# yglbgyx/DS-GAN

Hardware: AMD Instinct MI355X
Metric: 256×256 paired imgs/sec (G+D step) at 1/2/4/8 MI355X; MS-SSIM Δ vs ref (higher is better)
Workload: dtype bf16; 1 GPU; DS-GAN optimize_parameters, MixConvNeXtML G + PatchGAN D + VGG16 perceptual + SSIM/L1/TV; global_batch=16, per_gpu_batch=16, parallelism=dp1, hip_graphs=True

## Files before the change

### ds-gan_amd/csrc/pconv.hip

```cpp
#include "common.h"
#include "lds_pitch.h"
#include <type_traits>
#include <stdlib.h>

namespace dsg {

typedef f32x16_t cf32x16;
typedef __attribute__((ext_vector_type(4))) unsigned int cu32x4;

struct PcArgs {
  const float* X; long x_bs;
  const unsigned short* Wb;
  float* Y; long y_bs;
  const float* bias;
  const float* gpre; long gpre_bs;
  int nb, K, M, H, W, Ho, Wo, pad;
  int tiles_w, tiles_h;
  int act, gact; float slope;
  int accumulate;
  float* ws; int kchunk;
};

constexpr int PC_STR = 40;

template <typename T16, int BM, int TH, int TW, int S, int KH, int KW>
__global__ __launch_bounds__(256, 2) void pconv_kernel(PcArgs g) {
  typedef hx8<T16> cbf16x8;
  constexpr int BN = TH * TW;
  static_assert(BN == 128, "128 output pixels per tile");
  constexpr int WM = 2, WN = 2, TM = BM / WM / 32, TN = BN / WN / 32;
  constexpr int PH = (TH - 1) * S + KH, PW = (TW - 1) * S + KW, PPIX = PH * PW;
  constexpr int PWP = S == 1 ? 32 : PW;
  static_assert(PWP >= PW, "patch pitch");
  constexpr int TAPS = KH * KW;
  constexpr int A_SZ = BM * PC_STR, P_SZ = PH * PWP * PC_STR;
  constexpr int A_ITEMS = BM * 4 / 256;
  constexpr int P_ITEMS = (PPIX * 4 + 255) / 256;
  __shared__ __attribute__((aligned(16))) T16 smem[2 * A_SZ + P_SZ];
  T16* Ps = smem + 2 * A_SZ;

  const int tid = threadIdx.x, lane = tid & 63, wave = __builtin_amdgcn_readfirstlane(tid >> 6);
  const int wm = wave / WN, wn = wave % WN;
  const int lr = lane & 31, lh = lane >> 5;

  const int mt = (g.M + BM - 1) / BM;
  int tile;
  {
    const int nwg = gridDim.x, id = blockIdx.x;
    const int xcd = id & 7, q = nwg >> 3, r = nwg & 7;
    tile = (xcd < r ? xcd * (q + 1) : r * (q + 1) + (xcd - r) * q) + (id >> 3);
  }
  const int m_t = tile % mt, rest0 = tile / mt;
  const int tpi = g.tiles_w * g.tiles_h;
  const int split = rest0 / (g.nb * tpi), rest = rest0 - split * (g.nb * tpi);
  const int bimg = rest / tpi, t_i = rest - bimg * tpi;
  const int m0 = m_t * BM;
  const int oh0 = (t_i / g.tiles_w) * TH, ow0 = (t_i % g.tiles_w) * TW;
  const int ih0 = oh0 * S - g.pad, iw0 = ow0 * S - g.pad;
  const int HW = g.H * g.W;
  const float* xb = g.X + (long)bimg * g.x_bs;

  int pbase[TN];
#pragma unroll
  for (int j = 0; j < TN; ++j) {
    const int n = wn * (BN / WN) + j * 32 + lr;
    pbase[j] = ((n / TW) * S * PWP + (n % TW) * S) * PC_STR + lh * 8;
  }

  cu32x4 ra[A_ITEMS];
  auto aload = [&](int tap, int k0) {
#pragma unroll
    for (int i = 0; i < A_ITEMS; ++i) {
      const int it = tid + i * 256, row = p80_row16(it), c8 = p80_slot16(it);
      const int m = m0 + row;
      ra[i] = m < g.M ? *reinterpret_cast<const cu32x4*>(g.Wb + ((long)tap * g.M + m) * g.K + k0 + c8 * 8)
                      : cu32x4{0u, 0u, 0u, 0u};
    }
  };
  auto astore = [&](int buf) {
    T16* As = smem + buf * A_SZ;
#pragma unroll
    for (int i = 0; i < A_ITEMS; ++i) {
      const int it = tid + i * 256;
      *reinterpret_cast<cu32x4*>(As + p80_row16(it) * PC_STR + p80_slot16(it) * 8) = ra[i];
    }
  };
  float rp[P_ITEMS][8];
  auto pload = [&](int k0) {
#pragma unroll
    for (int i = 0; i < P_ITEMS; ++i) {
      const int it = tid + i * 256;
      const int cg = it / PPIX, pix = it - cg * PPIX;
      const int pr = pix / PW, pc = pix - pr * PW;
      const int ih = ih0 + pr, iw = iw0 + pc;
      const bool in = it < PPIX * 4 && (unsigned)ih < (unsigned)g.H && (unsigned)iw < (unsigned)g.W;
      const float* src = xb + (long)(k0 + (in ? cg : 0) * 8) * HW + (in ? ih * g.W + iw : 0);
#pragma unroll
      for (int e = 0; e < 8; ++e) rp[i][e] = in ? src[(long)e * HW] : 0.f;
    }
  };
  auto pwrite = [&]() {
#pragma unroll
    for (int i = 0; i < P_ITEMS; ++i) {
      const int it = tid + i * 256;
      if (it < PPIX * 4) {
        const int cg = it / PPIX, pix = it - cg * PPIX;
        const int pr = pix / PW, pc = pix - pr * PW;
        cbf16x8 v;
#pragma unroll
        for (int e = 0; e < 8; ++e) v[e] = (T16)rp[i][e];
        *reinterpret_cast<cbf16x8*>(Ps + (pr * PWP + pc) * PC_STR + cg * 8) = v;
      }
    }
  };

  cf32x16 acc[TM][TN];
#pragma unroll
  for (int i = 0; i < TM; ++i) {
    float bv[16];
#pragma unroll
    for (int r = 0; r < 16; ++r) {
      const int m = m0 + wm * TM * 32 + i * 32 + (r & 3) + 8 * (r >> 2) + 4 * lh;
      bv[r] = (g.bias && !g.ws && m < g.M) ? g.bias[m] : 0.f;
    }
#pragma unroll
    for (int j = 0; j < TN; ++j)
#pragma unroll
      for (int r = 0; r < 16; ++r) acc[i][j][r] = bv[r];
  }

  const int kb0 = g.ws ? split * g.kchunk : 0;
  const int nkb = g.ws ? min(g.K / 32, kb0 + g.kchunk) : g.K / 32;
  int buf = 0;
  aload(0, kb0 * 32);
  pload(kb0 * 32);
  for (int kb = kb0; kb < nkb; ++kb) {
    const int k0 = kb * 32;
    __syncthreads();
    pwrite();
    astore(buf);
    __syncthreads();
    if (kb + 1 < nkb) pload(k0 + 32);
#pragma unroll 1
    for (int tap = 0; tap < TAPS; ++tap) {
      if (tap + 1 < TAPS) aload(tap + 1, k0);
      else if (kb + 1 < nkb) aload(0, k0 + 32);
      const T16* As = smem + buf * A_SZ;
      const int kh = tap / KW, kw = tap - (tap / KW) * KW;
      const int toff = (kh * PWP + kw) * PC_STR;
#pragma unroll
      for (int ks = 0; ks < 2; ++ks) {
        cbf16x8 af[TM], bfr[TN];
#pragma unroll
        for (int i = 0; i < TM; ++i)
          af[i] = *reinterpret_cast<const cbf16x8*>(As + (wm * TM * 32 + i * 32 + lr) * PC_STR + ks * 16 + lh * 8);
#pragma unroll
        for (int j = 0; j < TN; ++j)
          bfr[j] = *reinterpret_cast<const cbf16x8*>(Ps + pbase[j] + toff + ks * 16);
#pragma unroll
        for (int i = 0; i < TM; ++i)
#pragma unroll
          for (int j = 0; j < TN; ++j)
            acc[i][j] = mfma16(af[i], bfr[j], acc[i][j]);
      }
      if (tap + 1 < TAPS) {
        astore(buf ^ 1);
        __syncthreads();
        buf ^= 1;
      }
    }
  }

  const int HWo = g.Ho * g.Wo;
  if (g.ws) {
    float* wp = g.ws + ((long)split * g.nb + bimg) * g.M * HWo;
#pragma unroll
    for (int j = 0; j < TN; ++j) {
      const int n = wn * (BN / WN) + j * 32 + lr;
      const int oh = oh0 + n / TW, ow = ow0 + n % TW;
      if (oh >= g.Ho || ow >= g.Wo) continue;
      const long pofs = (long)oh * g.Wo + ow;
#pragma unroll
      for (int i = 0; i < TM; ++i)
#pragma unroll
        for (int r = 0; r < 16; ++r) {
          const int m = m0 + wm * TM * 32 + i * 32 + (r & 3) + 8 * (r >> 2) + 4 * lh;
          if (m < g.M) wp[(long)m * HWo + pofs] = acc[i][j][r];
        }
    }
    return;
  }
// ... 90 lines not shown
    for (long e = blockIdx.x * 256L + threadIdx.x; e < en.total; e += stride) Wb[e] = (T16)W[e];
    return;
  }
  const int Co = en.Co, Ci = en.Ci, KH = en.KH, KW = en.KW, mode = en.mode;
  const int M = mode == 0 ? Co : Ci, K = mode == 0 ? Ci : Co, T = KH * KW;
  const long pairs = (long)M * K, plane = pairs;
  for (long e = blockIdx.x * 256L + threadIdx.x; e < pairs; e += stride) {
    const int k = (int)(e % K), m = (int)(e / K);
    const int co = mode == 0 ? m : k, ci = mode == 0 ? k : m;
    const float* src = W + ((long)co * Ci + ci) * T;
    for (int tap = 0; tap < T; ++tap) {
      int kh = tap / KW, kw = tap - (tap / KW) * KW;
      if (mode == 1) { kh = KH - 1 - kh; kw = KW - 1 - kw; }
      Wb[(long)tap * plane + e] = (T16)src[kh * KW + kw];
    }
  }
}

constexpr int PC_TH = 8, PC_TW = 16;
static long pc_tiles(int nb, int M, int Ho, int Wo, int BM) {
  return (long)nb * ((Wo + PC_TW - 1) / PC_TW) * ((Ho + PC_TH - 1) / PC_TH) * ((M + BM - 1) / BM);
}

template <typename T16, int BM, int TH, int TW, int S, int KH, int KW>
static void pc_launch(PcArgs& g, int splits, hipStream_t st) {
  static_assert(TH == PC_TH && TW == PC_TW, "pc_tiles");
  g.tiles_w = (g.Wo + TW - 1) / TW;
  g.tiles_h = (g.Ho + TH - 1) / TH;
  const long tiles = pc_tiles(g.nb, g.M, g.Ho, g.Wo, BM);
  hipLaunchKernelGGL((pconv_kernel<T16, BM, TH, TW, S, KH, KW>), dim3((unsigned)(tiles * splits)), dim3(256), 0, st, g);
  if (splits > 1) {
    const long per = (long)g.nb * g.M * g.Ho * g.Wo;
    long blocks = (per + 255) / 256;
    if (blocks > 8192) blocks = 8192;
    hipLaunchKernelGGL(pconv_reduce_kernel, dim3((unsigned)blocks), dim3(256), 0, st, g, splits);
  }
}

template <typename T16, int BM>
static int pc_dispatch(PcArgs& g, int KH, int S, int splits, hipStream_t st) {
  if constexpr (BM <= 128) {
    if (KH == 3 && S == 1) { pc_launch<T16, BM, PC_TH, PC_TW, 1, 3, 3>(g, splits, st); return 0; }
    if (KH == 4 && S == 1) { pc_launch<T16, BM, PC_TH, PC_TW, 1, 4, 4>(g, splits, st); return 0; }
  }
  if (KH == 4 && S == 2) { pc_launch<T16, BM, PC_TH, PC_TW, 2, 4, 4>(g, splits, st); return 0; }
  return -1;
}

}

using namespace dsg;

extern "C" {

int dsgan_pconv_supported(int K, int KH, int KW, int stride) {
  if (K % 32 != 0 || K <= 0 || KH != KW) return 0;
  return (KH == 3 && stride == 1) || (KH == 4 && (stride == 1 || stride == 2));
}

int dsgan_conv_wtrans_bf16(const float* W, void* Wb, int Co, int Ci, int KH, int KW, int mode, hipStream_t st) {
  DSG_REQUIRE(W && Wb && mode >= 0 && mode <= 2, "dsgan_conv_wtrans_bf16: bad args");
  const long total = (long)KH * KW * Co * Ci;
  long blocks = (total + 255) / 256;
  if (blocks > 8192) blocks = 8192;
  with_half([&](auto* t_) {
    using T16 = std::remove_pointer_t<decltype(t_)>;
    hipLaunchKernelGGL((wtrans_bf16_kernel<T16>), dim3((unsigned)blocks), dim3(256), 0, st, W, (T16*)Wb, Co, Ci, KH, KW,
                       mode);
  });
  DSG_CHECK_LAUNCH();
  return 0;
}

int dsgan_wtrans_multi(const void* const* W, void* const* Wb, const int* desc, int n, hipStream_t st) {
  DSG_REQUIRE(W && Wb && desc && n >= 0, "dsgan_wtrans_multi: bad args");
  for (int i0 = 0; i0 < n; i0 += WT_MAXE) {
    WtList L{};
    const int ne = n - i0 < WT_MAXE ? n - i0 : WT_MAXE;
    long most = 1;
    for (int i = 0; i < ne; ++i) {
// ... 24 lines not shown

long dsgan_pconv_workspace(int nb, int K, int M, int Ho, int Wo) {
  if (K % 32 != 0 || K <= 0) return 0;
  const int bm = pc_bm(nb, M, Ho, Wo);
  int kc;
  const int S = max(pc_splits(pc_tiles(nb, M, Ho, Wo, bm), K / 32, &kc),
                    pc_splits(pc_tiles(nb, M, Ho, Wo, bm == 256 ? 128 : bm), K / 32, &kc));
  return S > 1 ? (long)S * nb * M * Ho * Wo : 0;
}

int dsgan_pconv_ws(const float* X, long x_bs, const void* Wb, const float* bias, float* Y, long y_bs,
                   const float* gpre, long gpre_bs, int nb, int K, int M, int H, int W, int Ho, int Wo,
                   int KH, int KW, int stride, int pad, int act, int gact, float slope, int accumulate,
                   float* ws, long ws_elems, hipStream_t st);

int dsgan_pconv(const float* X, long x_bs, const void* Wb, const float* bias, float* Y, long y_bs,
                const float* gpre, long gpre_bs, int nb, int K, int M, int H, int W, int Ho, int Wo,
                int KH, int KW, int stride, int pad, int act, int gact, float slope, int accumulate,
                hipStream_t st) {
  return dsgan_pconv_ws(X, x_bs, Wb, bias, Y, y_bs, gpre, gpre_bs, nb, K, M, H, W, Ho, Wo, KH, KW, stride, pad, act,
                        gact, slope, accumulate, nullptr, 0, st);
}

int dsgan_pconv_ws(const float* X, long x_bs, const void* Wb, const float* bias, float* Y, long y_bs,
                   const float* gpre, long gpre_bs, int nb, int K, int M, int H, int W, int Ho, int Wo,
                   int KH, int KW, int stride, int pad, int act, int gact, float slope, int accumulate,
                   float* ws, long ws_elems, hipStream_t st) {
  DSG_REQUIRE(X && Wb && Y && nb > 0 && M > 0 && Ho > 0 && Wo > 0, "dsgan_pconv: bad args");
  DSG_REQUIRE(dsgan_pconv_supported(K, KH, KW, stride), "dsgan_pconv: unsupported K=%d KH=%d KW=%d stride=%d", K, KH, KW, stride);
  DSG_REQUIRE(((uintptr_t)Wb & 15) == 0, "dsgan_pconv: Wb must be 16-byte aligned");
  DSG_REQUIRE((Ho - 1) * stride - pad + KH <= H + pad && (Wo - 1) * stride - pad + KW <= W + pad,
              "dsgan_pconv: output size inconsistent with input/pad");
  PcArgs g{};
  g.X = X; g.x_bs = x_bs; g.Wb = (const unsigned short*)Wb; g.Y = Y; g.y_bs = y_bs; g.bias = bias;
  g.gpre = gpre; g.gpre_bs = gpre_bs; g.nb = nb; g.K = K; g.M = M; g.H = H; g.W = W; g.Ho = Ho;
  g.Wo = Wo; g.pad = pad; g.act = act; g.gact = gact; g.slope = slope; g.accumulate = accumulate;
  const int bm0 = pc_bm(nb, M, Ho, Wo);
  const int bm = bm0 == 256 ? (stride == 2 ? 256 : 128) : bm0;
  int kc = 0;
  const int splits = ws ? pc_splits(pc_tiles(nb, M, Ho, Wo, bm), K / 32, &kc) : 1;
  g.ws = splits > 1 ? ws : nullptr;
  g.kchunk = kc;
  DSG_WS(splits > 1 ? (long)splits * nb * M * Ho * Wo : 0, ws, ws_elems, "dsgan_pconv (dsgan_pconv_workspace)");
  const int rc = with_half([&](auto* t_) {
    using T16 = std::remove_pointer_t<decltype(t_)>;
    return bm == 256 ? pc_dispatch<T16, 256>(g, KH, stride, splits, st)
           : bm == 128 ? pc_dispatch<T16, 128>(g, KH, stride, splits, st)
                       : pc_dispatch<T16, 64>(g, KH, stride, splits, st);
  });
  DSG_REQUIRE(rc == 0, "dsgan_pconv: no kernel for KH=%d stride=%d", KH, stride);
  DSG_CHECK_LAUNCH();
  return 0;
}

}
```

### ds-gan_amd/dsgan_hip/_lib.py

```python
import ctypes
import os

import torch

_HERE = os.path.dirname(os.path.abspath(__file__))
LIB_PATH = os.environ.get("DSGAN_HIP_LIB", os.path.join(_HERE, "libdsgan_hip.so"))

P = ctypes.c_void_p
L = ctypes.c_long
I = ctypes.c_int
F = ctypes.c_float
D = ctypes.c_double
S = ctypes.c_void_p

SIGNATURES = {
    "dsgan_abi_version": [],
    "dsgan_set_half_type": [ctypes.c_int],
    "dsgan_amp_parts": [],
    "dsgan_amp_check": [P, L, P, P, F, F, I, S],
    "dsgan_adam_amp": [P, P, P, P, L, D, D, D, D, P, S],
    "dsgan_get_half_type": [],
    "dsgan_clear_launch_error": [],
    "dsgan_ktimer": [I],
    "dsgan_ktimer_read": [P, I],
# ... 14 lines not shown
    "dsgan_pw_dgrad_io_ws": [P, I, P, L, I, P, L, I, P, L, I, I, I, I, I, P, L, S],
    "dsgan_pw_fd_workspace": [I, I, I, I, I],
    "dsgan_wtrans_multi": [P, P, P, I, S],
    "dsgan_pw_tune": [I, I],
    "dsgan_pw_f32_supported": [I, I, I, I, L, L, P, P],
    "dsgan_pw_f32_wgrad_workspace": [I, I, I, I],
    "dsgan_pw_gemm_f32": [I, P, L, P, L, P, L, P, P, L, I, I, I, I, I, I, I, I, F, P, L, S],
    "dsgan_mlp_supported": [I, I, I],
    "dsgan_mlp_fwd": [P, L, I, P, P, P, P, P, L, I, I, I, I, I, S],
    "dsgan_mlp_bwd": [P, L, I, P, L, P, P, P, P, L, P, P, P, I, I, I, I, S],
    "dsgan_mlp_wgrad_workspace": [I, I, I, I],
    "dsgan_mlp_wgrad": [P, L, I, P, L, P, P, P, P, P, P, P, L, I, I, I, I, S],
    "dsgan_mlp_tune": [I, I],
    "dsgan_colsum": [P, I, I, P, S],
    "dsgan_split_defer": [I],
    "dsgan_split_pending": [],
    "dsgan_split_flush": [S],
    "dsgan_f32_to_bf16": [P, P, L, S],
    "dsgan_pconv_supported": [I, I, I, I],
    "dsgan_conv_wtrans_bf16": [P, P, I, I, I, I, I, S],
    "dsgan_pconv": [P, L, P, P, P, L, P, L] + [I] * 13 + [F, I, S],
    "dsgan_pconv_workspace": [I] * 5,
    "dsgan_pconv_ws": [P, L, P, P, P, L, P, L] + [I] * 13 + [F, I, P, L, S],
    "dsgan_pw_small_supported": [I, I, I, L, L],
    "dsgan_pw_small": [P, L, P, I, I, P, P, L, P, L] + [I] * 8 + [F, S],
    "dsgan_pw_small2": [P, L, P, I, I, P, L, P, I, P, P, L, P, L] + [I] * 8 + [F, S],
    "dsgan_pconvt_supported": [I, I, I, I],
    "dsgan_pconvt": [P, L, P, P, P, L, P, L] + [I] * 11 + [F, I, S],
    "dsgan_wconv_supported": [I, I, I, I],
    "dsgan_wconv_workspace": [I, I, I, I, I, I, I],
    "dsgan_wconv": [P, L, P, L, P, P, L] + [I] * 11 + [S],
    "dsgan_wconv_db": [P, L, P, L, P, P, P, L] + [I] * 11 + [S],
    "dsgan_wconv_xh": [P, L, P, L, P, P, L] + [I] * 11 + [S],
    "dsgan_conv_wtrans": [P, P, I, I, I, I, I, I, I, I, I, S],
    "dsgan_tconv": [P, L, P, P, P, L, P, L] + [I] * 9 + [P, P] + [I] * 7 + [F, S],
    "dsgan_tconv_workspace": [I] * 6,
    "dsgan_tconv_ws": [P, L, P, P, P, L, P, L] + [I] * 9 + [P, P] + [I] * 7 + [F, I, P, L, S],
    "dsgan_tconv_ws_xh": [P, L, P, P, P, L, P, L] + [I] * 9 + [P, P] + [I] * 7 + [F, P, L, S],
    "dsgan_conv_small_out": [P, L, P, L, L, L, L, P, P, L] + [I] * 13 + [S],
    "dsgan_conv_small_in": [P, L, P, L, L, L, L, P, P, L] + [I] * 13 + [F, I, S],
    "dsgan_conv_wgrad_small_workspace": [I] * 7,
    "dsgan_conv_wgrad_small": [P, L, P, L, P] + [I] * 11 + [P, L, S],
    "dsgan_thin3_supported": [I, I, I, L, L],
    "dsgan_pgstem_supported": [I] * 4,
    "dsgan_pgstem_fwd": [P, L, P, P, P, L] + [I] * 5 + [F, S],
    "dsgan_pgstem_wgrad_workspace": [I] * 5,
# ... 123 lines not shown
```

### ds-gan_amd/dsgan_hip/functional.py

```python
import contextlib
import os
import math

import ctypes

import torch

from . import _lib
from ._lib import call, ptr, stream


def wsa(t):
    if t is not None and _DEFER_KEEP[0] is not None:
        _DEFER_CAND.append(t)
    return (ptr(t), t.numel() if t is not None else 0)


DEFER_SPLITS = [os.environ.get("DSGAN_DEFER_SPLITS", "1") != "0"]
_DEFER_KEEP = [None]
_DEFER_CAND = []


def _defer_hook(queued):
    if queued and _DEFER_KEEP[0] is not None:
# ... 334 lines not shown
            and bool(_lib.load().dsgan_pw_small_supported(K, M, P, xbs, ybs)))


PGLAST = [True]


def _pglast_ok(Cout, Cin, KH, KW, stride, pad, H, W, w):
    return (PGLAST[0] and Cout == 1 and KH == 4 and KW == 4 and stride == 1 and pad == 1 and w.dim() == 4
            and w.is_contiguous() and bool(_lib.load().dsgan_pglast_supported(Cin, H, W)))


def _thin3_ok(M, H, W, bs_small, bs_big, t_small, t_big):
    return (t_small.data_ptr() % 16 == 0 and t_big.data_ptr() % 16 == 0
            and bool(_lib.load().dsgan_thin3_supported(M, H, W, bs_small, bs_big)))


def _pconv_ok(K, KH, KW, stride):
    return _is16() and bool(_lib.load().dsgan_pconv_supported(K, KH, KW, stride))


def _pconv(x, xbs, wb, b, y, ybs, N, K, M, H, W, Ho, Wo, KH, KW, stride, pad, act, gpre, gbs, gact, accumulate):
    nws = _lib.load().dsgan_pconv_workspace(N, K, M, Ho, Wo)
    ws = torch.empty(nws, device=x.device, dtype=torch.float32) if nws > 0 else None
    call("dsgan_pconv_ws", ptr(x), xbs, ptr(wb), ptr(b), ptr(y), ybs, ptr(gpre), gbs, N, K, M, H, W, Ho, Wo, KH, KW,
         stride, pad, ACT[act], ACT[gact], LRELU_SLOPE, int(accumulate), *wsa(ws), stream())


def conv_fwd_raw(x, w, b, stride, pad, act=None, out=None, pre=None, accumulate=False, xact=None):
    x, xbs = nchw(x)
    N, Cin, H, W = x.shape
    Cout, Cin_w, KH, KW = w.shape if w.dim() == 4 else (w.shape[0], w.shape[1], 1, 1)
    if Cin_w != Cin:
        raise ValueError("conv: input has %d channels, weight expects %d" % (Cin, Cin_w))
    Ho = (H + 2 * pad - KH) // stride + 1
    Wo = (W + 2 * pad - KW) // stride + 1
    y = out if out is not None else _empty(N, Cout, Ho, Wo, x)
    y, ybs = nchw(y)
    pbs = 0
    if pre is not None:
        pre, pbs = nchw(pre)
    e0 = IGEMM_TIMER.begin()
    fam = "igemm_kernel"
    if (KH == 3 and KW == 3 and stride == 1 and pad == 1 and act is None and pre is None and xact is None
            and w.is_contiguous() and _thin3_ok(Cout, H, W, ybs, xbs, y, x)):
        fam = "thin3_kernel"
        call("dsgan_thin3_fwd", ptr(x), xbs, ptr(w), ptr(b), ptr(y), ybs, N, Cin, Cout, H, W, int(accumulate),
             stream())
    elif KH == 1 and KW == 1 and stride == 1 and pad == 0 and pre is None and _pws_ok(Cin, Cout, H * W, xbs, ybs, x, y):
# ... 8 lines not shown
    elif Cout <= 8 and act is None and pre is None and xact is None:
        fam = "small_out_kernel"
        call("dsgan_conv_small_out", ptr(x), xbs, ptr(w), Cin * KH * KW, KH * KW, KW, 1, ptr(b), ptr(y), ybs,
             N, Cin, Cout, H, W, Ho, Wo, KH, KW, stride, pad, 0, int(accumulate), stream())
    elif Cin * KH * KW <= 36 and Cout >= 16 and pre is None and xact is None and act in (None, "relu", "lrelu"):
        fam = "small_in_kernel"
        call("dsgan_conv_small_in", ptr(x), xbs, ptr(w), Cin * KH * KW, KH * KW, KW, 1, ptr(b), ptr(y), ybs,
             N, Cin, Cout, H, W, Ho, Wo, KH, KW, stride, pad, 0, ACT[act], LRELU_SLOPE, int(accumulate), stream())
    elif KH == 1 and KW == 1 and stride == 1 and pad == 0 and _pw_ok(0, Cout, Cin, H * W, 0, xbs, w.data_ptr(), x.data_ptr()):
        fam = "pwgemm_kernel"
        if xact is None and _pw_io_ok(Cin, H * W, xbs, ybs, x, y, pre, pbs):
            call("dsgan_pw_fwd_io_ws", ptr(bf16_weight(w)), 1, ptr(x), xbs, 0, ptr(y), ybs, 0, ptr(pre), pbs, 0,
                 ptr(b), Cout, Cin, H * W, N, ACT[act], int(accumulate), LRELU_SLOPE,
                 *wsa(_pw_fd_ws(0, Cout, Cin, H * W, N, x)), stream())
        else:
            call("dsgan_pw_gemm", 0, ptr(w), 0, ptr(x), xbs, ptr(y), ybs, ptr(b), ptr(pre), pbs, None, 0,
                 Cout, N * H * W, Cin, H * W, N, ACT[act], 0, ACT[xact], int(accumulate), LRELU_SLOPE,
                 *wsa(_pw_fd_ws(0, Cout, Cin, H * W, N, x)), stream())
    elif (KH == 1 and KW == 1 and stride == 1 and pad == 0 and pre is None and xact is None
          and _pwf_ok(0, Cout, Cin, H * W, 0, xbs, w.data_ptr(), x.data_ptr())):
        fam = "pwf32_kernel"
        call("dsgan_pw_gemm_f32", 0, ptr(w), 0, ptr(x), xbs, ptr(y), ybs, ptr(b), None, 0, Cout, N * H * W, Cin,
             H * W, N, ACT[act], 0, int(accumulate), LRELU_SLOPE, None, 0, stream())
    elif w.dim() == 4 and pre is None and xact is None and _pconv_ok(Cin, KH, KW, stride):
        fam = "pconv_kernel"
        _pconv(x, xbs, _wtrans_bf16(w, 0), b, y, ybs, N, Cin, Cout, H, W, Ho, Wo, KH, KW, stride, pad, act,
               None, 0, None, accumulate)
    elif (_is16() and w.dim() == 4 and (KH > 1 or KW > 1) and Cin % 32 == 0
          and pre is None and not accumulate and xact is None and KH * KW <= 16):
        fam = "tconv_kernel"
        wt = _wtrans_bf16(w, 0) if Cin % 8 == 0 else _wtrans(w, 0)
        taps = [(kh - pad, kw - pad) for kh in range(KH) for kw in range(KW)]
        _tconv(x, xbs, wt, b, y, ybs, None, 0, N, Cin, Cout, H, W, Ho, Wo, stride, taps, Ho, Wo, 1, 0, 0,
               act, None)
    else:
        call("dsgan_conv_fwd", ptr(x), xbs, ptr(w), ptr(b), ptr(y), ybs, ptr(pre), pbs, N, Cin, H, W,
             Cout, KH, KW, stride, pad, Ho, Wo, ACT[act], LRELU_SLOPE, int(accumulate), ACT[xact], _prec(),
             stream())
    IGEMM_TIMER.end(e0, _conv_flops(N, Cin, Cout, KH, KW, Ho, Wo), ("fwd", N, Cin, H, W, Cout, KH, stride), fam,
                    _nb(x, w, b, y, pre) + (_nb(y) if accumulate else 0.0))
    return y


def conv_dgrad_raw(dy, w, x_shape, stride, pad, bias=None, act=None, gpre=None, gact=None,
                   out=None, accumulate=False):
    dy, dybs = nchw(dy)
    N, Cin, H, W = x_shape
# ... 981 lines not shown
            res = None
        else:
            x, w, t, mean, rstd, res = ctx.saved_tensors
        N, Ci, Hi, Wi = x.shape
        Co, H, W = t.shape[1], t.shape[2], t.shape[3]
        HW = H * W
        dyt, dybs = nchw(dy[:, :Co] if ctx.cat else dy)
        t4, tbs = nchw(t)
        rbs = 0
        if res is not None:
            res, rbs = nchw(res)
        want_dres = res is not None and ctx.needs_input_grad[3]
        dres = _empty(N, Co, H, W, t) if want_dres else None
        dth = torch.empty((N, Co, H, W), device=t.device, dtype=half_dtype())
        psum = torch.empty(N * Co, device=t.device, dtype=torch.float32)
        e0 = AUX_TIMER.begin()
        call("dsgan_instnorm_bwd_h", ptr(dyt), dybs, ptr(t4), tbs, ptr(res), rbs, ptr(mean), ptr(rstd), ptr(dth),
             Co * HW, ptr(psum), ptr(dres), Co * HW, N, Co, HW, _in_act(ctx.act), LRELU_SLOPE, IN_EPS, stream())
        AUX_TIMER.end(e0, 0.0, ("in_bwd_h", N, Co, H, W, ctx.act, res is not None), "instnorm",
                      _nb(dyt, t4, res, dres) + _nb(dth))
        dx = None
        if ctx.needs_input_grad[0]:
            dx = _empty(N, Ci, Hi, Wi, x)
            taps = [(kh - 1, kw - 1) for kh in range(3) for kw in range(3)]
            dh = (ctypes.c_int * 9)(*[q[0] for q in taps])
            dw = (ctypes.c_int * 9)(*[q[1] for q in taps])
            nws = _lib.load().dsgan_tconv_workspace(N, Co, Ci, Hi, Wi, 9)
            ws = torch.empty(nws, device=t.device, dtype=torch.float32) if nws > 0 else None
            e0 = IGEMM_TIMER.begin()
            call("dsgan_tconv_ws_xh", ptr(dth), Co * HW, ptr(_wtrans_bf16(w, 0)), None, ptr(dx), Ci * Hi * Wi, None,
                 0, N, Co, Ci, H, W, Hi, Wi, 2, 9, ctypes.cast(dh, ctypes.c_void_p), ctypes.cast(dw, ctypes.c_void_p),
                 Hi, Wi, 1, 0, 0, 0, 0, LRELU_SLOPE, *wsa(ws), stream())
            IGEMM_TIMER.end(e0, _conv_flops(N, Co, Ci, 3, 3, Hi, Wi), ("fwd", N, Co, H, W, Ci, 3, 2), "tconv_kernel",
                            _nb(dth, dx) + 2.0 * w.numel())
        gw = _grad_buf(ctx.w_ref) if ctx.needs_input_grad[1] else None
        if gw is not None:
            x4, xbs = nchw(x)
            ws = torch.empty(_lib.load().dsgan_wconv_workspace(N, Co, Ci, Hi, Wi, 3, 3), device=t.device,
                             dtype=torch.float32)
            e0 = IGEMM_TIMER.begin()
            call("dsgan_wconv_xh", ptr(x4), xbs, ptr(dth), Co * HW, ptr(gw), *wsa(ws), N, Co, Ci, H, W, Hi, Wi, 3, 3,
                 2, 1, stream())
            IGEMM_TIMER.end(e0, _conv_flops(N, Co, Ci, 3, 3, Hi, Wi), ("wgrad", N, Co, H, W, Ci, 3, 2), "wconv_kernel",
                            _nb(x4, dth, gw))
        gb = _grad_buf(ctx.b_ref) if (ctx.has_b and ctx.needs_input_grad[2]) else None
        if gb is not None:
# ... 674 lines not shown
```

### include/dsgan_hip.h

```cpp
#ifndef DSGAN_HIP_H
#define DSGAN_HIP_H

#include <hip/hip_runtime.h>

#ifdef __cplusplus
extern "C" {
#endif

int dsgan_abi_version(void);
const char* dsgan_last_error_string(void);
int dsgan_set_plan_only(int on);
long dsgan_last_ws_need(void);
int dsgan_set_half_type(int t);
int dsgan_get_half_type(void);
int dsgan_clear_launch_error(void);
int dsgan_ktimer(int on);
int dsgan_ktimer_read(float* ms, int max);

int dsgan_conv_fwd(const float* x, long x_bs, const float* w, const float* bias, float* y,
                   long y_bs, float* ypre, long ypre_bs, int N, int Cin, int H, int W, int Cout,
                   int KH, int KW, int stride, int pad, int Ho, int Wo, int act, float slope,
                   int accumulate, int xact, int prec, hipStream_t stream);
int dsgan_conv_dgrad(const float* dy, long dy_bs, const float* w, const float* bias, float* dx,
                     long dx_bs, float* ypre, long ypre_bs, const float* gpre, long gpre_bs,
// ... 109 lines not shown
                   const float* gpre, long gpre_bs, int nb, int K, int M, int Hin, int Win, int Hout,
                   int Wout, int stride, int ntaps, const int* dh, const int* dw, int Hdst, int Wdst,
                   int os, int ph, int pw, int act, int gact, float slope, int wt_bf16, float* ws,
                   long ws_elems, hipStream_t stream);
int dsgan_tconv_ws_xh(const void* Xh, long x_bs, const void* Wt, const float* bias, float* Y, long y_bs,
                      const float* gpre, long gpre_bs, int nb, int K, int M, int Hin, int Win, int Hout,
                      int Wout, int stride, int ntaps, const int* dh, const int* dw, int Hdst, int Wdst,
                      int os, int ph, int pw, int act, int gact, float slope, float* ws, long ws_elems,
                      hipStream_t stream);

int dsgan_pconv_supported(int K, int KH, int KW, int stride);
int dsgan_conv_wtrans_bf16(const float* W, void* Wb, int Co, int Ci, int KH, int KW, int mode,
                           hipStream_t stream);
int dsgan_wtrans_multi(const void* const* W, void* const* Wb, const int* desc, int n, hipStream_t stream);
int dsgan_pconv(const float* X, long x_bs, const void* Wb, const float* bias, float* Y, long y_bs,
                const float* gpre, long gpre_bs, int nb, int K, int M, int H, int W, int Ho, int Wo,
                int KH, int KW, int stride, int pad, int act, int gact, float slope, int accumulate,
                hipStream_t stream);
long dsgan_pconv_workspace(int nb, int K, int M, int Ho, int Wo);
int dsgan_pconv_ws(const float* X, long x_bs, const void* Wb, const float* bias, float* Y, long y_bs,
                   const float* gpre, long gpre_bs, int nb, int K, int M, int H, int W, int Ho, int Wo,
                   int KH, int KW, int stride, int pad, int act, int gact, float slope, int accumulate,
                   float* ws, long ws_elems, hipStream_t stream);

int dsgan_pw_small_supported(int K, int M, int P, long x_bs, long y_bs);
int dsgan_pw_small(const float* X, long x_bs, const float* W, int wm, int wk, const float* bias, float* Y,
                   long y_bs, const float* G, long g_bs, int nb, int K, int M, int P, int act, int xact,
                   int gact, int accumulate, float slope, hipStream_t stream);
int dsgan_pw_small2(const float* X, long x_bs, const float* W, int wm, int wk, const float* X2,
                    long x2_bs, const float* W2, int K2, const float* bias, float* Y, long y_bs,
                    const float* G, long g_bs, int nb, int K, int M, int P, int act, int xact, int gact,
                    int accumulate, float slope, hipStream_t stream);

int dsgan_pconvt_supported(int K, int KS, int stride, int pad);
int dsgan_pconvt(const float* X, long x_bs, const void* Wb, const float* bias, float* Y, long y_bs,
                 const float* gpre, long gpre_bs, int nb, int K, int M, int Hi, int Wi, int Ho, int Wo,
                 int KS, int stride, int pad, int gact, float slope, int accumulate, hipStream_t stream);

int dsgan_wconv_supported(int C, int KH, int KW, int stride);
long dsgan_wconv_workspace(int nb, int C, int M, int Ho, int Wo, int KH, int KW);
int dsgan_wconv(const float* D, long d_bs, const float* X, long x_bs, float* dw, float* ws, long ws_elems,
                int nb, int C, int M, int H, int W, int Ho, int Wo, int KH, int KW, int stride, int pad,
                hipStream_t stream);
int dsgan_wconv_db(const float* D, long d_bs, const float* X, long x_bs, float* dw, float* db, float* ws,
                   long ws_elems, int nb, int C, int M, int H, int W, int Ho, int Wo, int KH, int KW, int stride,
                   int pad, hipStream_t stream);
// ... 152 lines not shown
```

Before: 651.1 img/s.

## Add 3x3 stride-2 patch-conv path with 16-bit vectorized input staging

Extends the patch-tile implicit-GEMM conv kernel to 3x3 stride-2 convolutions, and routes the conv-transpose data-gradient and eligible forward 3x3/s2 convs through it. A new 16-bit input variant stages rows with 128-bit vector loads and register shuffles instead of per-element gathers. A three-deep register ring prefetches weight slices across taps, with the unrolled tap loop. The aim is to replace the slower generic tap-gather path and cut global load instruction count, at the cost of more registers and template instantiations.

```diff
diff --git a/ds-gan_amd/csrc/pconv.hip b/ds-gan_amd/csrc/pconv.hip
--- a/ds-gan_amd/csrc/pconv.hip
+++ b/ds-gan_amd/csrc/pconv.hip
@@ -9,7 +9,7 @@
 typedef __attribute__((ext_vector_type(4))) unsigned int cu32x4;
 
 struct PcArgs {
-  const float* X; long x_bs;
+  const void* X; long x_bs;
   const unsigned short* Wb;
   float* Y; long y_bs;
   const float* bias;
@@ -23,9 +23,11 @@
 
 constexpr int PC_STR = 40;
 
-template <typename T16, int BM, int TH, int TW, int S, int KH, int KW>
+template <typename T16, int BM, int TH, int TW, int S, int KH, int KW, bool XH = false, bool VEC = false>
 __global__ __launch_bounds__(256, 2) void pconv_kernel(PcArgs g) {
   typedef hx8<T16> cbf16x8;
+  typedef std::conditional_t<XH, unsigned short, float> XT;
+  static_assert(!VEC || (XH && S == 2 && KH == 3 && KW == 3 && TW == 16), "row staging: 16-bit 3x3 stride 2");
   constexpr int BN = TH * TW;
   static_assert(BN == 128, "128 output pixels per tile");
   constexpr int WM = 2, WN = 2, TM = BM / WM / 32, TN = BN / WN / 32;
@@ -36,6 +38,8 @@
   constexpr int A_SZ = BM * PC_STR, P_SZ = PH * PWP * PC_STR;
   constexpr int A_ITEMS = BM * 4 / 256;
   constexpr int P_ITEMS = (PPIX * 4 + 255) / 256;
+  constexpr int V_ITEMS = (PH * 32 + 255) / 256;
+  constexpr int GI = VEC ? 1 : P_ITEMS, VI = VEC ? V_ITEMS : 1;
   __shared__ __attribute__((aligned(16))) T16 smem[2 * A_SZ + P_SZ];
   T16* Ps = smem + 2 * A_SZ;
 
@@ -58,7 +62,7 @@
   const int oh0 = (t_i / g.tiles_w) * TH, ow0 = (t_i % g.tiles_w) * TW;
   const int ih0 = oh0 * S - g.pad, iw0 = ow0 * S - g.pad;
   const int HW = g.H * g.W;
-  const float* xb = g.X + (long)bimg * g.x_bs;
+  const XT* xb = (const XT*)g.X + (long)bimg * g.x_bs;
 
   int pbase[TN];
 #pragma unroll
@@ -67,51 +71,120 @@
     pbase[j] = ((n / TW) * S * PWP + (n % TW) * S) * PC_STR + lh * 8;
   }
 
-  cu32x4 ra[A_ITEMS];
-  auto aload = [&](int tap, int k0) {
+  constexpr int AD = VEC ? 3 : 1;
+  static_assert(TAPS % AD == 0 && TAPS > AD, "slice ring");
+  cu32x4 ra[AD][A_ITEMS];
+  auto aload_s = [&](int slot, int tap, int k0) {
 #pragma unroll
     for (int i = 0; i < A_ITEMS; ++i) {
       const int it = tid + i * 256, row = p80_row16(it), c8 = p80_slot16(it);
       const int m = m0 + row;
-      ra[i] = m < g.M ? *reinterpret_cast<const cu32x4*>(g.Wb + ((long)tap * g.M + m) * g.K + k0 + c8 * 8)
-                      : cu32x4{0u, 0u, 0u, 0u};
-    }
-  };
-  auto astore = [&](int buf) {
+      ra[slot][i] = m < g.M ? *reinterpret_cast<const cu32x4*>(g.Wb + ((long)tap * g.M + m) * g.K + k0 + c8 * 8)
+                            : cu32x4{0u, 0u, 0u, 0u};
+    }
+  };
+  auto astore_s = [&](int buf, int slot) {
     T16* As = smem + buf * A_SZ;
 #pragma unroll
     for (int i = 0; i < A_ITEMS; ++i) {
       const int it = tid + i * 256;
-      *reinterpret_cast<cu32x4*>(As + p80_row16(it) * PC_STR + p80_slot16(it) * 8) = ra[i];
-    }
-  };
-  float rp[P_ITEMS][8];
-  auto pload = [&](int k0) {
-#pragma unroll
-    for (int i = 0; i < P_ITEMS; ++i) {
+      *reinterpret_cast<cu32x4*>(As + p80_row16(it) * PC_STR + p80_slot16(it) * 8) = ra[slot][i];
+    }
+  };
+  auto aload = [&](int tap, int k0) { aload_s(0, tap, k0); };
+  auto astore = [&](int buf) { astore_s(buf, 0); };
+  XT rp[GI][8];
+  auto pload_g = [&](int k0) {
+#pragma unroll
+    for (int i = 0; i < GI; ++i) {
       const int it = tid + i * 256;
       const int cg = it / PPIX, pix = it - cg * PPIX;
       const int pr = pix / PW, pc = pix - pr * PW;
       const int ih = ih0 + pr, iw = iw0 + pc;
       const bool in = it < PPIX * 4 && (unsigned)ih < (unsigned)g.H && (unsigned)iw < (unsigned)g.W;
-      const float* src = xb + (long)(k0 + (in ? cg : 0) * 8) * HW + (in ? ih * g.W + iw : 0);
-#pragma unroll
-      for (int e = 0; e < 8; ++e) rp[i][e] = in ? src[(long)e * HW] : 0.f;
-    }
-  };
-  auto pwrite = [&]() {
-#pragma unroll
-    for (int i = 0; i < P_ITEMS; ++i) {
+      const XT* src = xb + (long)(k0 + (in ? cg : 0) * 8) * HW + (in ? ih * g.W + iw : 0);
+#pragma unroll
+      for (int e = 0; e < 8; ++e) rp[i][e] = in ? src[(long)e * HW] : (XT)0;
+    }
+  };
+  auto pwrite_g = [&]() {
+#pragma unroll
+    for (int i = 0; i < GI; ++i) {
       const int it = tid + i * 256;
       if (it < PPIX * 4) {
         const int cg = it / PPIX, pix = it - cg * PPIX;
         const int pr = pix / PW, pc = pix - pr * PW;
         cbf16x8 v;
 #pragma unroll
-        for (int e = 0; e < 8; ++e) v[e] = (T16)rp[i][e];
+        for (int e = 0; e < 8; ++e) {
+          if constexpr (XH) v[e] = __builtin_bit_cast(T16, rp[i][e]);
+          else v[e] = (T16)rp[i][e];
+        }
         *reinterpret_cast<cbf16x8*>(Ps + (pr * PWP + pc) * PC_STR + cg * 8) = v;
       }
     }
+  };
+  cu32x4 rv[VI][4];
+  unsigned short rl[4];
+  auto pload_v = [&](int k0) {
+#pragma unroll
+    for (int i = 0; i < VI; ++i) {
+      const int it = tid + i * 256;
+      const int c = it & 3, cg = (it >> 2) & 7, pr = it >> 5;
+      const int ih = ih0 + pr, iw = iw0 + 1 + 8 * c;
+      const bool in = pr < PH && (unsigned)ih < (unsigned)g.H && iw < g.W;
+      const XT* src = xb + (long)(k0 + cg * 4) * HW + (in ? ih * g.W + iw : 0);
+#pragma unroll
+      for (int e = 0; e < 4; ++e)
+        rv[i][e] = in ? *reinterpret_cast<const cu32x4*>(src + (long)e * HW) : cu32x4{0u, 0u, 0u, 0u};
+    }
+    {
+      const int cg = tid & 7, pr = tid >> 3;
+      const int ih = ih0 + pr;
+      const bool in = pr < PH && (unsigned)ih < (unsigned)g.H && iw0 >= 0;
+      const XT* src = xb + (long)(k0 + cg * 4) * HW + (in ? ih * g.W + iw0 : 0);
+#pragma unroll
+      for (int e = 0; e < 4; ++e) rl[e] = in ? src[(long)e * HW] : (XT)0;
+    }
+  };
+  auto pwrite_v = [&]() {
+    typedef __attribute__((ext_vector_type(2))) unsigned int cu32x2;
+#pragma unroll
+    for (int i = 0; i < VI; ++i) {
+      const int it = tid + i * 256;
+      const int c = it & 3, cg = (it >> 2) & 7, pr = it >> 5;
+      if (pr < PH) {
+        cu32x4 r[4];
+#pragma unroll
+        for (int e = 0; e < 4; ++e) {
+          const cu32x4 u = rv[i][e];
+          const cu32x4 t = (c & 1) ? cu32x4{u[1], u[2], u[3], u[0]} : u;
+          r[e] = (c & 2) ? cu32x4{t[2], t[3], t[0], t[1]} : t;
+        }
+        T16* row = Ps + (pr * PWP + 1 + 8 * c) * PC_STR + cg * 4;
+#pragma unroll
+        for (int d = 0; d < 4; ++d) {
+          T16* dst = row + 2 * ((d + c) & 3) * PC_STR;
+          *reinterpret_cast<cu32x2*>(dst) =
+              cu32x2{(r[0][d] & 0xffffu) | (r[1][d] << 16), (r[2][d] & 0xffffu) | (r[3][d] << 16)};
+          *reinterpret_cast<cu32x2*>(dst + PC_STR) =
+              cu32x2{(r[0][d] >> 16) | (r[1][d] & 0xffff0000u), (r[2][d] >> 16) | (r[3][d] & 0xffff0000u)};
+        }
+      }
+    }
+    if (tid < PH * 8) {
+      const int cg = tid & 7, pr = tid >> 3;
+      *reinterpret_cast<cu32x2*>(Ps + pr * PWP * PC_STR + cg * 4) =
+          cu32x2{(unsigned)rl[0] | ((unsigned)rl[1] << 16), (unsigned)rl[2] | ((unsigned)rl[3] << 16)};
+    }
+  };
+  auto pload = [&](int k0) {
+    if constexpr (VEC) pload_v(k0);
+    else pload_g(k0);
+  };
+  auto pwrite = [&]() {
+    if constexpr (VEC) pwrite_v();
+    else pwrite_g();
   };
 
   cf32x16 acc[TM][TN];
@@ -132,41 +205,72 @@
   const int kb0 = g.ws ? split * g.kchunk : 0;
   const int nkb = g.ws ? min(g.K / 32, kb0 + g.kchunk) : g.K / 32;
   int buf = 0;
-  aload(0, kb0 * 32);
-  pload(kb0 * 32);
-  for (int kb = kb0; kb < nkb; ++kb) {
-    const int k0 = kb * 32;
-    __syncthreads();
-    pwrite();
-    astore(buf);
-    __syncthreads();
-    if (kb + 1 < nkb) pload(k0 + 32);
+  auto tap_mma = [&](int tap) {
+    const T16* As = smem + buf * A_SZ;
+    const int kh = tap / KW, kw = tap - (tap / KW) * KW;
+    const int toff = (kh * PWP + kw) * PC_STR;
+#pragma unroll
+    for (int ks = 0; ks < 2; ++ks) {
+      cbf16x8 af[TM], bfr[TN];
+#pragma unroll
+      for (int i = 0; i < TM; ++i)
+        af[i] = *reinterpret_cast<const cbf16x8*>(As + (wm * TM * 32 + i * 32 + lr) * PC_STR + ks * 16 + lh * 8);
+#pragma unroll
+      for (int j = 0; j < TN; ++j)
+        bfr[j] = *reinterpret_cast<const cbf16x8*>(Ps + pbase[j] + toff + ks * 16);
+#pragma unroll
+      for (int i = 0; i < TM; ++i)
+#pragma unroll
+        for (int j = 0; j < TN; ++j)
+          acc[i][j] = mfma16(af[i], bfr[j], acc[i][j]);
+    }
+  };
+  if constexpr (AD > 1) {
+    constexpr int PT = TAPS - 1 - AD - 1;
+#pragma unroll
+    for (int s = 0; s < AD; ++s) aload_s(s, s, kb0 * 32);
+    pload(kb0 * 32);
+    for (int kb = kb0; kb < nkb; ++kb) {
+      const int k0 = kb * 32;
+      __syncthreads();
+      pwrite();
+      astore_s(buf, 0);
+      __syncthreads();
+      aload_s(0, AD, k0);
+#pragma unroll
+      for (int tap = 0; tap < TAPS; ++tap) {
+        tap_mma(tap);
+        if (tap + 1 < TAPS) {
+          const int slot = (tap + 1) % AD, nt = tap + 1 + AD;
+          astore_s(buf ^ 1, slot);
+          if (nt < TAPS) aload_s(slot, nt, k0);
+          if (tap == PT && kb + 1 < nkb) pload(k0 + 32);
+          if (nt >= TAPS && kb + 1 < nkb) aload_s(slot, nt - TAPS, k0 + 32);
+          __syncthreads();
+          buf ^= 1;
+        }
+      }
+    }
+  } else {
+    aload(0, kb0 * 32);
+    pload(kb0 * 32);
+    for (int kb = kb0; kb < nkb; ++kb) {
+      const int k0 = kb * 32;
+      __syncthreads();
+      pwrite();
+      astore(buf);
+      __syncthreads();
+      if (kb + 1 < nkb) pload(k0 + 32);
 #pragma unroll 1
-    for (int tap = 0; tap < TAPS; ++tap) {
-      if (tap + 1 < TAPS) aload(tap + 1, k0);
-      else if (kb + 1 < nkb) aload(0, k0 + 32);
-      const T16* As = smem + buf * A_SZ;
-      const int kh = tap / KW, kw = tap - (tap / KW) * KW;
-      const int toff = (kh * PWP + kw) * PC_STR;
-#pragma unroll
-      for (int ks = 0; ks < 2; ++ks) {
-        cbf16x8 af[TM], bfr[TN];
-#pragma unroll
-        for (int i = 0; i < TM; ++i)
-          af[i] = *reinterpret_cast<const cbf16x8*>(As + (wm * TM * 32 + i * 32 + lr) * PC_STR + ks * 16 + lh * 8);
-#pragma unroll
-        for (int j = 0; j < TN; ++j)
-          bfr[j] = *reinterpret_cast<const cbf16x8*>(Ps + pbase[j] + toff + ks * 16);
-#pragma unroll
-        for (int i = 0; i < TM; ++i)
-#pragma unroll
-          for (int j = 0; j < TN; ++j)
-            acc[i][j] = mfma16(af[i], bfr[j], acc[i][j]);
-      }
-      if (tap + 1 < TAPS) {
-        astore(buf ^ 1);
-        __syncthreads();
-        buf ^= 1;
+      for (int tap = 0; tap < TAPS; ++tap) {
+        if (tap + 1 < TAPS) aload(tap + 1, k0);
+        else if (kb + 1 < nkb) aload(0, k0 + 32);
+        tap_mma(tap);
+        if (tap + 1 < TAPS) {
+          astore(buf ^ 1);
+          __syncthreads();
+          buf ^= 1;
+        }
       }
     }
   }
@@ -303,13 +407,14 @@
   return (long)nb * ((Wo + PC_TW - 1) / PC_TW) * ((Ho + PC_TH - 1) / PC_TH) * ((M + BM - 1) / BM);
 }
 
-template <typename T16, int BM, int TH, int TW, int S, int KH, int KW>
+template <typename T16, int BM, int TH, int TW, int S, int KH, int KW, bool XH = false, bool VEC = false>
 static void pc_launch(PcArgs& g, int splits, hipStream_t st) {
   static_assert(TH == PC_TH && TW == PC_TW, "pc_tiles");
   g.tiles_w = (g.Wo + TW - 1) / TW;
   g.tiles_h = (g.Ho + TH - 1) / TH;
   const long tiles = pc_tiles(g.nb, g.M, g.Ho, g.Wo, BM);
-  hipLaunchKernelGGL((pconv_kernel<T16, BM, TH, TW, S, KH, KW>), dim3((unsigned)(tiles * splits)), dim3(256), 0, st, g);
+  hipLaunchKernelGGL((pconv_kernel<T16, BM, TH, TW, S, KH, KW, XH, VEC>), dim3((unsigned)(tiles * splits)), dim3(256), 0,
+                     st, g);
   if (splits > 1) {
     const long per = (long)g.nb * g.M * g.Ho * g.Wo;
     long blocks = (per + 255) / 256;
@@ -325,7 +430,16 @@
     if (KH == 4 && S == 1) { pc_launch<T16, BM, PC_TH, PC_TW, 1, 4, 4>(g, splits, st); return 0; }
   }
   if (KH == 4 && S == 2) { pc_launch<T16, BM, PC_TH, PC_TW, 2, 4, 4>(g, splits, st); return 0; }
+  if (KH == 3 && S == 2) { pc_launch<T16, BM, PC_TH, PC_TW, 2, 3, 3>(g, splits, st); return 0; }
   return -1;
+}
+
+template <typename T16, int BM>
+static int pc_dispatch_xh(PcArgs& g, int KH, int S, int splits, bool vec, hipStream_t st) {
+  if (KH != 3 || S != 2) return -1;
+  if (vec) pc_launch<T16, BM, PC_TH, PC_TW, 2, 3, 3, true, true>(g, splits, st);
+  else pc_launch<T16, BM, PC_TH, PC_TW, 2, 3, 3, true, false>(g, splits, st);
+  return 0;
 }
 
 }
@@ -336,7 +450,7 @@
 
 int dsgan_pconv_supported(int K, int KH, int KW, int stride) {
   if (K % 32 != 0 || K <= 0 || KH != KW) return 0;
-  return (KH == 3 && stride == 1) || (KH == 4 && (stride == 1 || stride == 2));
+  return (KH == 3 && (stride == 1 || stride == 2)) || (KH == 4 && (stride == 1 || stride == 2));
 }
 
 int dsgan_conv_wtrans_bf16(const float* W, void* Wb, int Co, int Ci, int KH, int KW, int mode, hipStream_t st) {
@@ -407,15 +521,19 @@
                         gact, slope, accumulate, nullptr, 0, st);
 }
 
-int dsgan_pconv_ws(const float* X, long x_bs, const void* Wb, const float* bias, float* Y, long y_bs,
-                   const float* gpre, long gpre_bs, int nb, int K, int M, int H, int W, int Ho, int Wo,
-                   int KH, int KW, int stride, int pad, int act, int gact, float slope, int accumulate,
-                   float* ws, long ws_elems, hipStream_t st) {
+}
+
+static int pconv_impl(const void* X, long x_bs, const void* Wb, const float* bias, float* Y, long y_bs,
+                      const float* gpre, long gpre_bs, int nb, int K, int M, int H, int W, int Ho, int Wo,
+                      int KH, int KW, int stride, int pad, int act, int gact, float slope, int accumulate,
+                      int x_half, float* ws, long ws_elems, hipStream_t st) {
   DSG_REQUIRE(X && Wb && Y && nb > 0 && M > 0 && Ho > 0 && Wo > 0, "dsgan_pconv: bad args");
   DSG_REQUIRE(dsgan_pconv_supported(K, KH, KW, stride), "dsgan_pconv: unsupported K=%d KH=%d KW=%d stride=%d", K, KH, KW, stride);
+  DSG_REQUIRE(!x_half || (KH == 3 && stride == 2), "dsgan_pconv_ws_xh: 3x3 stride 2 only (KH=%d stride=%d)", KH, stride);
   DSG_REQUIRE(((uintptr_t)Wb & 15) == 0, "dsgan_pconv: Wb must be 16-byte aligned");
   DSG_REQUIRE((Ho - 1) * stride - pad + KH <= H + pad && (Wo - 1) * stride - pad + KW <= W + pad,
               "dsgan_pconv: output size inconsistent with input/pad");
+  DSG_REQUIRE((long)H * W < (1L << 31), "dsgan_pconv: plane too large");
   PcArgs g{};
   g.X = X; g.x_bs = x_bs; g.Wb = (const unsigned short*)Wb; g.Y = Y; g.y_bs = y_bs; g.bias = bias;
   g.gpre = gpre; g.gpre_bs = gpre_bs; g.nb = nb; g.K = K; g.M = M; g.H = H; g.W = W; g.Ho = Ho;
@@ -427,8 +545,17 @@
   g.ws = splits > 1 ? ws : nullptr;
   g.kchunk = kc;
   DSG_WS(splits > 1 ? (long)splits * nb * M * Ho * Wo : 0, ws, ws_elems, "dsgan_pconv (dsgan_pconv_workspace)");
+  bool vec = false;
+  if (x_half) {
+    const char* e = getenv("DSGAN_PCONV_GATHER");
+    vec = !(e && *e && *e != '0') && pad == 1 && W % 8 == 0 && x_bs % 8 == 0 && ((uintptr_t)X & 15) == 0;
+  }
   const int rc = with_half([&](auto* t_) {
     using T16 = std::remove_pointer_t<decltype(t_)>;
+    if (x_half)
+      return bm == 256 ? pc_dispatch_xh<T16, 256>(g, KH, stride, splits, vec, st)
+             : bm == 128 ? pc_dispatch_xh<T16, 128>(g, KH, stride, splits, vec, st)
+                         : pc_dispatch_xh<T16, 64>(g, KH, stride, splits, vec, st);
     return bm == 256 ? pc_dispatch<T16, 256>(g, KH, stride, splits, st)
            : bm == 128 ? pc_dispatch<T16, 128>(g, KH, stride, splits, st)
                        : pc_dispatch<T16, 64>(g, KH, stride, splits, st);
@@ -438,4 +565,22 @@
   return 0;
 }
 
-}
+extern "C" {
+
+int dsgan_pconv_ws(const float* X, long x_bs, const void* Wb, const float* bias, float* Y, long y_bs,
+                   const float* gpre, long gpre_bs, int nb, int K, int M, int H, int W, int Ho, int Wo,
+                   int KH, int KW, int stride, int pad, int act, int gact, float slope, int accumulate,
+                   float* ws, long ws_elems, hipStream_t st) {
+  return pconv_impl(X, x_bs, Wb, bias, Y, y_bs, gpre, gpre_bs, nb, K, M, H, W, Ho, Wo, KH, KW, stride, pad, act, gact,
+                    slope, accumulate, 0, ws, ws_elems, st);
+}
+
+int dsgan_pconv_ws_xh(const void* Xh, long x_bs, const void* Wb, const float* bias, float* Y, long y_bs,
+                      const float* gpre, long gpre_bs, int nb, int K, int M, int H, int W, int Ho, int Wo,
+                      int KH, int KW, int stride, int pad, int act, int gact, float slope, int accumulate,
+                      float* ws, long ws_elems, hipStream_t st) {
+  return pconv_impl(Xh, x_bs, Wb, bias, Y, y_bs, gpre, gpre_bs, nb, K, M, H, W, Ho, Wo, KH, KW, stride, pad, act, gact,
+                    slope, accumulate, 1, ws, ws_elems, st);
+}
+
+}
diff --git a/ds-gan_amd/dsgan_hip/_lib.py b/ds-gan_amd/dsgan_hip/_lib.py
--- a/ds-gan_amd/dsgan_hip/_lib.py
+++ b/ds-gan_amd/dsgan_hip/_lib.py
@@ -60,6 +60,7 @@
     "dsgan_pconv": [P, L, P, P, P, L, P, L] + [I] * 13 + [F, I, S],
     "dsgan_pconv_workspace": [I] * 5,
     "dsgan_pconv_ws": [P, L, P, P, P, L, P, L] + [I] * 13 + [F, I, P, L, S],
+    "dsgan_pconv_ws_xh": [P, L, P, P, P, L, P, L] + [I] * 13 + [F, I, P, L, S],
     "dsgan_pw_small_supported": [I, I, I, L, L],
     "dsgan_pw_small": [P, L, P, I, I, P, P, L, P, L] + [I] * 8 + [F, S],
     "dsgan_pw_small2": [P, L, P, I, I, P, L, P, I, P, P, L, P, L] + [I] * 8 + [F, S],
diff --git a/ds-gan_amd/dsgan_hip/functional.py b/ds-gan_amd/dsgan_hip/functional.py
--- a/ds-gan_amd/dsgan_hip/functional.py
+++ b/ds-gan_amd/dsgan_hip/functional.py
@@ -380,8 +380,13 @@
 def _pconv(x, xbs, wb, b, y, ybs, N, K, M, H, W, Ho, Wo, KH, KW, stride, pad, act, gpre, gbs, gact, accumulate):
     nws = _lib.load().dsgan_pconv_workspace(N, K, M, Ho, Wo)
     ws = torch.empty(nws, device=x.device, dtype=torch.float32) if nws > 0 else None
-    call("dsgan_pconv_ws", ptr(x), xbs, ptr(wb), ptr(b), ptr(y), ybs, ptr(gpre), gbs, N, K, M, H, W, Ho, Wo, KH, KW,
-         stride, pad, ACT[act], ACT[gact], LRELU_SLOPE, int(accumulate), *wsa(ws), stream())
+    call("dsgan_pconv_ws" if x.dtype == torch.float32 else "dsgan_pconv_ws_xh", ptr(x), xbs, ptr(wb), ptr(b), ptr(y),
+         ybs, ptr(gpre), gbs, N, K, M, H, W, Ho, Wo, KH, KW, stride, pad, ACT[act], ACT[gact], LRELU_SLOPE,
+         int(accumulate), *wsa(ws), stream())
+
+
+def _convt_dgrad_pconv(K, W):
+    return W % 8 == 0 and _pconv_ok(K, 3, 3, 2)
 
 
 def conv_fwd_raw(x, w, b, stride, pad, act=None, out=None, pre=None, accumulate=False, xact=None):
@@ -436,7 +441,8 @@
         fam = "pwf32_kernel"
         call("dsgan_pw_gemm_f32", 0, ptr(w), 0, ptr(x), xbs, ptr(y), ybs, ptr(b), None, 0, Cout, N * H * W, Cin,
              H * W, N, ACT[act], 0, int(accumulate), LRELU_SLOPE, None, 0, stream())
-    elif w.dim() == 4 and pre is None and xact is None and _pconv_ok(Cin, KH, KW, stride):
+    elif (w.dim() == 4 and pre is None and xact is None and _pconv_ok(Cin, KH, KW, stride)
+          and ((KH, stride) != (3, 2) or (pad == 1 and _convt_dgrad_pconv(Cin, W)))):
         fam = "pconv_kernel"
         _pconv(x, xbs, _wtrans_bf16(w, 0), b, y, ybs, N, Cin, Cout, H, W, Ho, Wo, KH, KW, stride, pad, act,
                None, 0, None, accumulate)
@@ -1464,6 +1470,13 @@
         dx = None
         if ctx.needs_input_grad[0]:
             dx = _empty(N, Ci, Hi, Wi, x)
+        if dx is not None and _convt_dgrad_pconv(Co, W):
+            e0 = IGEMM_TIMER.begin()
+            _pconv(dth, Co * HW, _wtrans_bf16(w, 0), None, dx, Ci * Hi * Wi, N, Co, Ci, H, W, Hi, Wi, 3, 3, 2, 1, None,
+                   None, 0, None, False)
+            IGEMM_TIMER.end(e0, _conv_flops(N, Co, Ci, 3, 3, Hi, Wi), ("fwd", N, Co, H, W, Ci, 3, 2), "pconv_kernel",
+                            _nb(dth, dx) + 2.0 * w.numel())
+        elif dx is not None:
             taps = [(kh - 1, kw - 1) for kh in range(3) for kw in range(3)]
             dh = (ctypes.c_int * 9)(*[q[0] for q in taps])
             dw = (ctypes.c_int * 9)(*[q[1] for q in taps])
diff --git a/include/dsgan_hip.h b/include/dsgan_hip.h
--- a/include/dsgan_hip.h
+++ b/include/dsgan_hip.h
@@ -155,6 +155,10 @@
                    const float* gpre, long gpre_bs, int nb, int K, int M, int H, int W, int Ho, int Wo,
                    int KH, int KW, int stride, int pad, int act, int gact, float slope, int accumulate,
                    float* ws, long ws_elems, hipStream_t stream);
+int dsgan_pconv_ws_xh(const void* Xh, long x_bs, const void* Wb, const float* bias, float* Y, long y_bs,
+                      const float* gpre, long gpre_bs, int nb, int K, int M, int H, int W, int Ho, int Wo,
+                      int KH, int KW, int stride, int pad, int act, int gact, float slope, int accumulate,
+                      float* ws, long ws_elems, hipStream_t stream);
 
 int dsgan_pw_small_supported(int K, int M, int P, long x_bs, long y_bs);
 int dsgan_pw_small(const float* X, long x_bs, const float* W, int wm, int wk, const float* bias, float* Y,
```

Result: no change. 654.4 img/s, median of 6 (+0.5%).
